# HKU-BAL/MegaPath-Nano

Hardware: AMD Instinct MI355X
Metric: Gbp/min ONT reads aligned+species-assigned vs RefSeq, 1/2/4/8 MI355X (higher is better)
Workload: dtype int32

## Files before the change

### megapath_nano_amd/csrc/map_kernels.h

```cpp
#pragma once
#include "mpn_common.h"
#include "map_types.h"

#include <type_traits>

namespace mpn {

__device__ __forceinline__ uint64_t hash64m(uint64_t key, uint64_t mask) {
    key = (~key + (key << 21)) & mask;
    key = key ^ key >> 24;
    key = ((key + (key << 3)) + (key << 8)) & mask;
    key = key ^ key >> 14;
    key = ((key + (key << 2)) + (key << 4)) & mask;
    key = key ^ key >> 28;
    key = (key + (key << 31)) & mask;
    return key;
}

constexpr int SKETCH_FAST_MAX_W = 32;

template <bool HASH64>
__device__ __forceinline__ uint64_t sketch_hash(uint64_t key, uint64_t mask) {
    if (HASH64) return hash64m(key, mask);
    uint32_t h = (uint32_t)key;
// ... 653 lines not shown
                int lo = 0, hi = 63;
#pragma unroll
                for (int step = 0; step < 6; ++step) {
                    const int mid = (lo + hi + 1) >> 1;
                    if (g[mid] <= p) lo = mid; else hi = mid - 1;
                }
                const uint64_t r = pos[ps[lo] + (p - g[lo])];
                const uint64_t y = yy[lo];
                const uint32_t q_pos = (uint32_t)y, q_span = (uint32_t)(y >> 32) & 0xff;
                const uint32_t rpos = (uint32_t)r >> 1;
                u128 a;
                if ((r & 1) == (q_pos & 1)) {
                    a.x = (r & 0xffffffff00000000ULL) | rpos;
                    a.y = (uint64_t)q_span << 32 | q_pos >> 1;
                } else {
                    a.x = 1ULL << 63 | (r & 0xffffffff00000000ULL) | rpos;
                    a.y = (uint64_t)q_span << 32 | (uint32_t)(qlen - ((int32_t)(q_pos >> 1) + 1 - (int32_t)q_span) - 1);
                }
                a.y |= y & (1ULL << 42);
                anchors[out + __popcll(km & ((1ULL << lane) - 1))] = a;
            }
            out += __popcll(km);
        }
        __builtin_amdgcn_wave_barrier();
    }
}

template <int NY>
__device__ __forceinline__ uint32_t sort_digit(const u128 &r, int pass) {
    return pass < NY ? (uint32_t)(r.y >> (8 * pass)) & 0xff : (uint32_t)(r.x >> (8 * (pass - NY))) & 0xff;
}

constexpr int WORK_SLOTS = 256;
__device__ __forceinline__ void add_work(unsigned long long *work, unsigned long long n) {
    if (work) atomicAdd(&work[blockIdx.x & (WORK_SLOTS - 1)], n);
}

struct SegSortLds {
    uint32_t hist[256], bins[256], wcnt[4][256];
    int skip;
};

template <int NY>
__device__ __forceinline__ void wg_radix_sort(SegSortLds &L, u128 *__restrict__ data, u128 *__restrict__ tmp, int64_t n,
                                              unsigned long long *__restrict__ work) {
    const int tid = threadIdx.x, lane = tid & 63, wv = tid >> 6;
    u128 *src = data, *dst = tmp;
    for (int pass = 0; pass < NY + 8; ++pass) {
        L.hist[tid] = 0;
        __syncthreads();
        for (int64_t i = tid; i < n; i += 256) atomicAdd(&L.hist[sort_digit<NY>(src[i], pass)], 1u);
        __syncthreads();
        if (tid == 0) L.skip = 0;
        __syncthreads();
        if (L.hist[tid] == (uint32_t)n) L.skip = 1;
        __syncthreads();
        if (L.skip) { __syncthreads(); continue; }
        if (tid == 0) add_work(work, (unsigned long long)n);
        {
            uint32_t v = L.hist[tid];
            L.bins[tid] = v;
            __syncthreads();
            for (int d = 1; d < 256; d <<= 1) {
                uint32_t a = tid >= d ? L.bins[tid - d] : 0;
                __syncthreads();
                L.bins[tid] += a;
// ... 559 lines not shown
                    max_f = best;
                    max_j = j0 - wl;
                }
                if (!tile_in_ring && elig && pj >= 0) {
                    if (pj >= win_lo) wt[pj & M] = i;
                    else { t[pj] = i; gmark = true; }
                }
                if (brk < 64) done = true;
                if (__ballot(gmark)) __builtin_amdgcn_fence(__ATOMIC_RELEASE, "workgroup");
                MPN_LDS_FENCE();
            }
            int32_t vprev = 0;
            if (max_j >= 0) vprev = max_j >= win_lo ? wv[max_j & M] : v[max_j];
            const int32_t vi = (max_j >= 0 && vprev > max_f) ? vprev : max_f;
            if (lane == li) { rf = max_f; rp = max_j >= 0 ? max_j + rel : -1; rv = vi; }
            if (lane == 0) {
                const int sl = i & M;
                *reinterpret_cast<uint4 *>(&ring[sl]) = make_uint4(ri, (uint32_t)qi, (uint32_t)max_f, (uint32_t)max_j);
                wv[sl] = vi; wt[sl] = 0;
            }
            MPN_LDS_FENCE();
            if (li == 63 || i == n - 1) {
                const int32_t k = (i & ~63) + lane;
                if (k <= i) { f[k] = rf; p[k] = rp; v[k] = rv; }
                const uint32_t carry = (uint32_t)__builtin_amdgcn_readlane((int)cx, 63);
                cx = (uint32_t)wave_scan_add((int)nstep) + carry; cx64 = nx64; cyl = nyl; cyh = nyh;
            }
        }
        __builtin_amdgcn_fence(__ATOMIC_RELEASE, "workgroup");
        __syncthreads();
    }
}

__global__ __launch_bounds__(64) void chain_ends_kernel(const int64_t *__restrict__ anchor_off, int n_reads, ChainParams cp,
                                                        const int32_t *__restrict__ F, const int32_t *__restrict__ P,
                                                        int32_t *__restrict__ T, const int32_t *__restrict__ V,
                                                        uint64_t *__restrict__ U, int32_t *__restrict__ n_ends) {
    const int lane = threadIdx.x;
    for (int read = blockIdx.x; read < n_reads; read += gridDim.x) {
        const int64_t base = anchor_off[read];
        const int64_t n = anchor_off[read + 1] - base;
        const int32_t *f = F + base, *p = P + base, *v = V + base;
        int32_t *t = T + base;
        uint64_t *u = U + base;
        for (int64_t i = lane; i < n; i += 64) t[i] = 0;
        __builtin_amdgcn_fence(__ATOMIC_RELEASE, "workgroup");
        __syncthreads();
        for (int64_t i = lane; i < n; i += 64) if (p[i] >= 0) t[p[i]] = 1;
        __builtin_amdgcn_fence(__ATOMIC_RELEASE, "workgroup");
        __syncthreads();
        int cnt = 0;
        for (int64_t i0 = 0; i0 < n; i0 += 64) {
            const int64_t i = i0 + lane;
            bool is_end = i < n && t[i] == 0 && v[i] >= cp.min_sc;
            uint64_t val = 0;
            if (is_end) {
                int64_t j = i;
                while (j >= 0 && f[j] < v[j]) j = p[j];
                if (j < 0) j = i;
                val = (uint64_t)(uint32_t)f[j] << 32 | (uint64_t)j;
            }
            const unsigned long long m = __ballot(is_end);
            if (is_end) u[cnt + __popcll(m & ((1ULL << lane) - 1))] = val;
            cnt += __popcll(m);
        }
        if (lane == 0) n_ends[read] = cnt;
        __syncthreads();
    }
}

__global__ __launch_bounds__(256) void chain_sort_ends_kernel(uint64_t *__restrict__ U, uint64_t *__restrict__ Utmp,
                                                              const int64_t *__restrict__ anchor_off,
                                                              const int32_t *__restrict__ n_ends, int n_reads) {
    __shared__ uint32_t hist[256];
    __shared__ uint32_t bins[256];
    __shared__ uint32_t wcnt[4][256];
    __shared__ int s_skip;
    const int tid = threadIdx.x, lane = tid & 63, wv = tid >> 6;
    for (int read = blockIdx.x; read < n_reads; read += gridDim.x) {
        const int64_t base = anchor_off[read];
        const int n = n_ends[read];
        if (n < 2) continue;
        uint64_t *src = U + base, *dst = Utmp + base;
        for (int pass = 0; pass < 8; ++pass) {
            hist[tid] = 0;
            __syncthreads();
            for (int i = tid; i < n; i += 256) atomicAdd(&hist[(uint32_t)(~src[i] >> (8 * pass)) & 0xff], 1u);
            __syncthreads();
            if (tid == 0) s_skip = 0;
            __syncthreads();
            if (hist[tid] == (uint32_t)n) s_skip = 1;
            __syncthreads();
            if (s_skip) { __syncthreads(); continue; }
            {
                uint32_t v = hist[tid];
                bins[tid] = v;
                __syncthreads();
                for (int d = 1; d < 256; d <<= 1) {
                    uint32_t a = tid >= d ? bins[tid - d] : 0;
                    __syncthreads();
                    bins[tid] += a;
                    __syncthreads();
                }
                uint32_t excl = bins[tid] - v;
                __syncthreads();
                bins[tid] = excl;
                __syncthreads();
            }
            for (int t0 = 0; t0 < n; t0 += 256) {
                const int i = t0 + tid;
                const bool act = i < n;
                uint64_t r = 0;
                uint32_t dg = 0;
                if (act) { r = src[i]; dg = (uint32_t)(~r >> (8 * pass)) & 0xff; }
                wcnt[0][tid] = 0; wcnt[1][tid] = 0; wcnt[2][tid] = 0; wcnt[3][tid] = 0;
                __syncthreads();
                unsigned long long same = __ballot(act);
#pragma unroll
                for (int b = 0; b < 8; ++b) {
                    unsigned long long m = __ballot((dg >> b) & 1);
                    same &= ((dg >> b) & 1) ? m : ~m;
                }
                const uint32_t rank = __popcll(same & ((1ULL << lane) - 1));
                if (act && rank == 0) wcnt[wv][dg] = __popcll(same);
                __syncthreads();
                if (act) {
                    uint32_t o = bins[dg] + rank;
                    for (int w2 = 0; w2 < wv; ++w2) o += wcnt[w2][dg];
                    dst[o] = r;
                }
                __syncthreads();
                bins[tid] += wcnt[0][tid] + wcnt[1][tid] + wcnt[2][tid] + wcnt[3][tid];
                __syncthreads();
            }
            uint64_t *sw = src; src = dst; dst = sw;
            __threadfence_block();
            __syncthreads();
        }
        if (src != U + base) for (int i = tid; i < n; i += 256) U[base + i] = src[i];
        __syncthreads();
    }
}

constexpr int BT_PAR_MIN = 16;

__global__ __launch_bounds__(64) void chain_backtrack_kernel(const u128 *__restrict__ anchors, const int64_t *__restrict__ anchor_off,
                                                             int n_reads, ChainParams cp, const int32_t *__restrict__ F,
                                                             const int32_t *__restrict__ P, int32_t *__restrict__ T,
                                                             int32_t *__restrict__ V, uint64_t *__restrict__ U,
                                                             const int32_t *__restrict__ n_ends, u128 *__restrict__ B,
                                                             uint64_t *__restrict__ Uc, unsigned long long *__restrict__ used,
                                                             int64_t *__restrict__ u_pos, int64_t *__restrict__ b_pos,
                                                             int32_t *__restrict__ n_chain, int64_t *__restrict__ n_chained,
                                                             ChainRec *__restrict__ Rc, int par_min) {
    __shared__ int s_k;
    __shared__ unsigned long long s_up, s_bp;
    const int lane = threadIdx.x;
    for (int read = blockIdx.x; read < n_reads; read += gridDim.x) {
        const int64_t base = anchor_off[read];
        const int64_t n = anchor_off[read + 1] - base;
        const u128 *a = anchors + base;
        const int32_t *f = F + base, *p = P + base;
        int32_t *t = T + base, *v = V + base;
        uint64_t *u = U + base;
        const int n_u = n_ends[read];
        if (n_u >= par_min) {
            for (int64_t i = lane; i < n; i += 64) t[i] = 0x7fffffff;
            __builtin_amdgcn_fence(__ATOMIC_RELEASE, "agent");
            __syncthreads();
            for (int e0 = 0; e0 < n_u; e0 += 64) {
                const int e = e0 + lane;
                if (e < n_u) {
                    int32_t j = (int32_t)u[e];
                    while (j >= 0) { const int32_t nj = p[j]; if (atomicMin(&t[j], e) < e) break; j = nj; }
                }
            }
            __builtin_amdgcn_fence(__ATOMIC_ACQ_REL, "agent");
            __syncthreads();
            int k_run = 0, nv_run = 0;
            for (int e0 = 0; e0 < n_u; e0 += 64) {
                const int e = e0 + lane;
                int cnt = 0;
                if (e < n_u) {
                    const uint64_t ui = u[e];
                    int32_t j = p[(int32_t)ui];
                    cnt = 1;
                    while (j >= 0) { const int32_t tj = t[j], nj = p[j]; if (tj != e) break; ++cnt; j = nj; }
                    const bool keep = cnt >= cp.min_cnt && (j < 0 || (int32_t)(ui >> 32) - f[j] >= cp.min_sc);
                    if (!keep) cnt = 0;
                    v[e] = cnt;
                }
                k_run += __builtin_amdgcn_readlane(wave_scan_add(cnt > 0 ? 1 : 0), 63);
                nv_run += __builtin_amdgcn_readlane(wave_scan_add(cnt), 63);
// ... 78 lines not shown
        const int k = s_k;
        u128 *b = B + s_bp;
        uint64_t *uc = Uc + s_up;
        ChainRec *rc = Rc + s_up;
        int off = 0;
        for (int c = 0; c < k; ++c) {
            const int ni = (int32_t)u[c];
            int ml = 0, bl = 0;
            for (int j = lane; j < ni; j += 64) {
                const u128 cur = a[v[off + (ni - j - 1)]];
                b[off + j] = cur;
                const int span = (int)(cur.y >> 32 & 0xff);
                if (j == 0) { ml += span; bl += span; }
                else {
                    const u128 prev = a[v[off + (ni - j)]];
                    const int tl = (int32_t)cur.x - (int32_t)prev.x, ql = (int32_t)cur.y - (int32_t)prev.y;
                    bl += tl > ql ? tl : ql;
                    ml += tl > span && ql > span ? span : tl < ql ? tl : ql;
                }
            }
            ml = __builtin_amdgcn_readlane(wave_scan_add(ml), 63);
            bl = __builtin_amdgcn_readlane(wave_scan_add(bl), 63);
            if (lane == 0) {
                const u128 first = a[v[off + ni - 1]], last = a[v[off]];
                rc[c] = ChainRec{first.x, first.y, last.x, last.y, ml, bl};
            }
            off += ni;
        }
        for (int c = lane; c < k; c += 64) uc[c] = u[c];
        __syncthreads();
    }
}

__global__ __launch_bounds__(256) void idx_bucket_hist_kernel(const u128 *__restrict__ mz, int64_t n, int shift, unsigned long long *__restrict__ hist) {
    for (int64_t i = (int64_t)blockIdx.x * blockDim.x + threadIdx.x; i < n; i += (int64_t)gridDim.x * blockDim.x)
        atomicAdd(&hist[(mz[i].x >> 8) >> shift], 1ULL);
}

__global__ __launch_bounds__(256) void idx_bucket_scatter_kernel(const u128 *__restrict__ mz, int64_t n, int shift,
                                                                 unsigned long long *__restrict__ cursor, u128 *__restrict__ out) {
    for (int64_t i = (int64_t)blockIdx.x * blockDim.x + threadIdx.x; i < n; i += (int64_t)gridDim.x * blockDim.x) {
        u128 r = mz[i];
        r.x >>= 8;
        const unsigned long long p = atomicAdd(&cursor[r.x >> shift], 1ULL);
        out[p] = r;
    }
}

__global__ __launch_bounds__(256) void idx_flag_count_kernel(const u128 *__restrict__ rec, int64_t n, int64_t *__restrict__ block_cnt) {
    __shared__ int s[256];
    const int64_t base = (int64_t)blockIdx.x * 2048;
    int c = 0;
    for (int k = 0; k < 8; ++k) {
        const int64_t i = base + k * 256 + threadIdx.x;
        if (i < n && (i == 0 || rec[i].x != rec[i - 1].x)) ++c;
    }
    s[threadIdx.x] = c;
    __syncthreads();
    for (int d = 128; d; d >>= 1) { if (threadIdx.x < d) s[threadIdx.x] += s[threadIdx.x + d]; __syncthreads(); }
    if (threadIdx.x == 0) block_cnt[blockIdx.x] = s[0];
}

__global__ __launch_bounds__(256) void idx_emit_kernel(const u128 *__restrict__ rec, int64_t n, const int64_t *__restrict__ block_off,
                                                       uint64_t *__restrict__ keys, int64_t *__restrict__ key_off,
                                                       uint64_t *__restrict__ pos) {
    __shared__ int s[256];
// ... 77 lines not shown
```

### megapath_nano_amd/csrc/mapper.hip

```cpp
#include "map_kernels.h"
#include "mapper_internal.h"
#include "../../include/mpn_map.h"

#include <algorithm>
#include <mutex>
#include <string.h>
#include <time.h>
#include <sys/stat.h>
#include <string>
#include <vector>

namespace mpn {

hipError_t stream_sync(hipStream_t st) {
    struct Ev {
        hipEvent_t e = nullptr;
        ~Ev() { if (e) (void)hipEventDestroy(e); }
    };
    static thread_local Ev ev;
    hipError_t rc;
    if (!ev.e && (rc = hipEventCreateWithFlags(&ev.e, hipEventDisableTiming)) != hipSuccess) return rc;
    if ((rc = hipEventRecord(ev.e, st)) != hipSuccess) return rc;
    unsigned int us = 20;
    for (;;) {
// ... 189 lines not shown
int sketch_reads(int k, int w, int n, const uint8_t *d_seqs, const int64_t *d_off, const int32_t *d_len, const int32_t *h_len, ReadSketch &sk,
                 StreamLease &st) {
    EvTimer ev(st);
    sk.valid = false;
    if (sketch_device(d_seqs, d_off, d_len, h_len, n, k, w, 0, sk.mz_off, sk.mz, &sk.n_mz, st, &ev)) return -1;
    MPN_HIP_CHECK(stream_sync(st));
    ev.resolve();
    sk.k = k; sk.w = w; sk.valid = true;
    return 0;
}

int seed_chain_device(const mpn_index *idx, const mpn_map_opt *opt, int n, const uint8_t *d_seqs, const int64_t *d_off,
                      const int32_t *d_len, const int32_t *h_len, SeedChainOut &o, StreamLease &st, const ReadSketch *pre) {
    int64_t n_mz = 0;
    DevBuf<int64_t> mz_off;
    DevBuf<u128> mz;
    EvTimer ev(st);
    if (pre && pre->valid && pre->k == idx->k && pre->w == idx->w) {
        mz_off.p = pre->mz_off.p; mz_off.n = pre->mz_off.n; mz_off.owned = false;
        mz.p = pre->mz.p; mz.n = pre->mz.n; mz.owned = false;
        n_mz = pre->n_mz;
    } else if (sketch_device(d_seqs, d_off, d_len, h_len, n, idx->k, idx->w, 0, mz_off, mz, &n_mz, st, &ev)) return -1;
    g_stats[1] += n_mz;
    int32_t mid_occ = opt->mid_occ > 0 ? opt->mid_occ : mpn_index_mid_occ(idx, opt->mid_occ_frac);
    if (mid_occ > (1 << 25)) {
        const int32_t top = mpn_index_mid_occ(idx, 1e-30f);
        if (top > 0) mid_occ = std::min(mid_occ, top);
    }
    DevBuf<int32_t> occ;
    DevBuf<int64_t> pos_start, rel_off, full_off, n_blk, blk_base;
    DevBuf<unsigned long long> span_sum;
    {
        const size_t N = (size_t)n, o1 = (N + 1) * 8, o2 = o1 + N * 8, o3 = o2 + N * 8, o4 = o3 + N * 8, o5 = o4 + N * 4, o6 = (o5 + N * 4 + 7) & ~(size_t)7;
        o.tables_bytes = o6 + (size_t)(2 + WORK_SLOTS) * 8;
        if (o.tables.alloc(o.tables_bytes)) return -1;
        auto view = [&](auto &buf, size_t off, size_t count) { buf.release(); buf.p = reinterpret_cast<decltype(buf.p)>(o.tables.p + off); buf.n = count; buf.owned = false; };
        view(o.n_anchor, 0, N + 1); view(o.n_chained, o1, N); view(o.u_pos, o2, N); view(o.b_pos, o3, N);
        view(o.n_chain, o4, N); view(o.rep_len, o5, N); view(o.used, o6, 2 + WORK_SLOTS);
    }
    if (occ.alloc(n_mz) || pos_start.alloc(n_mz) || rel_off.alloc(n_mz) || full_off.alloc((size_t)n + 1) ||
        n_blk.alloc((size_t)n + 1) || blk_base.alloc((size_t)n + 1) || span_sum.alloc(n) || o.anchor_off.alloc((size_t)n + 1))
        return -1;
    if (n_mz > 0) {
        hipLaunchKernelGGL(seed_lookup_kernel, dim3(grid_1d(n_mz, 256)), dim3(256), 0, st, (const u128 *)idx->kv.p,
                           idx->n_keys, (const int64_t *)idx->bucket_start.p, idx->bucket_shift, mz.p, n_mz, mid_occ, occ.p, pos_start.p);
        MPN_HIP_CHECK(hipGetLastError());
        ev.mark(11, 35);
    }
    hipLaunchKernelGGL(seed_prefix_kernel, dim3(std::max(1, std::min(n, 256 * 32))), dim3(64), 0, st, mz.p, mz_off.p, n, occ.p, rel_off.p,
                       o.n_anchor.p, o.rep_len.p, span_sum.p, n_blk.p);
    MPN_HIP_CHECK(hipGetLastError());
    hipLaunchKernelGGL(scan_i64x2_kernel, dim3(2), dim3(1024), 0, st, (const int64_t *)o.n_anchor.p, full_off.p, n, (const int64_t *)n_blk.p, blk_base.p, n);
    MPN_HIP_CHECK(hipGetLastError());
    int64_t n_full = 0;
    if (read_i64(full_off.p + n, &n_full, st)) return -1;
    g_stats[2] += n_full;
    const int64_t nb_cap = n_mz / 64 + n + 1;
    DevBuf<unsigned long long> keep;
    DevBuf<int64_t> blk_kept, blk_off;
    DevBuf<int32_t> blk_read, order;
    DevBuf<unsigned int> next_read;
    DevBuf<unsigned int> n_list, seg_counters;
    DevBuf<unsigned long long> read_kept;
    if (next_read.alloc(4) || order.alloc(n) || keep.alloc((size_t)(n_full / 64 + nb_cap + 8)) || blk_kept.alloc((size_t)nb_cap + 1) || blk_off.alloc((size_t)nb_cap + 2) ||
        blk_read.alloc((size_t)nb_cap + 1) || n_list.alloc(4) || seg_counters.alloc(4) || read_kept.alloc(n))
        return -1;
    {
        ZeroList z{};
        zero_list_push(z, next_read.p, 4 * sizeof(unsigned int));
        zero_list_push(z, blk_kept.p, ((size_t)nb_cap + 1) * 8);
        zero_list_push(z, o.used.p, o.used.n * sizeof(unsigned long long));
// ... 77 lines not shown
                           (const unsigned int *)n_list.p, lists.cap[0], o.used.p + 2);
        hipLaunchKernelGGL(anchor_bitonic_list_kernel<BITONIC_MID>, dim3(256 * 4), dim3(256), 0, st, o.anchors.p, (const SortSeg *)lists.seg[1],
                           (const unsigned int *)n_list.p + 1, lists.cap[1], o.used.p + 2);
        hipLaunchKernelGGL(seg_sort_list_kernel<4>, dim3(256 * 4), dim3(256), 0, st, o.anchors.p, tmp.p, (const SortSeg *)lists.seg[2],
                           (const unsigned int *)n_list.p + 2, lists.cap[2], o.used.p + 2);
        MPN_HIP_CHECK(hipGetLastError());
        ev.mark(12, 49);
    }
    ChainParams cp;
    cp.max_dist_x = opt->max_gap; cp.max_dist_y = opt->max_gap; cp.bw = opt->bw; cp.max_skip = opt->max_chain_skip;
    cp.max_iter = opt->max_chain_iter; cp.min_cnt = opt->min_cnt; cp.min_sc = opt->min_chain_score;
    const int g = std::max(1, std::min(n, 256 * 32));
    const int64_t n_pieces = (n_a + COMPACT_PIECE - 1) / COMPACT_PIECE;
    DevBuf<int64_t> kept, piece_kept, piece_off;
    DevBuf<float> avg_qspan;
    if (kept.alloc((size_t)n + 1) || o.c_off.alloc((size_t)n + 1) || avg_qspan.alloc(n) || piece_kept.alloc((size_t)n_pieces + 1) ||
        piece_off.alloc((size_t)n_pieces + 1))
        return -1;
    const int gp = (int)std::max<int64_t>(1, std::min<int64_t>(n_pieces, 256 * 64));
    if (n_a > 0) {
        hipLaunchKernelGGL(anchor_compact_kernel<false>, dim3(gp), dim3(64), 0, st, (const u128 *)o.anchors.p, (const int64_t *)o.anchor_off.p, n, n_a,
                           cp.max_dist_x, cp.min_cnt, piece_kept.p, read_kept.p, (const int64_t *)nullptr, (u128 *)nullptr);
        MPN_HIP_CHECK(hipGetLastError());
    }
    hipLaunchKernelGGL(anchor_compact_finish_kernel, dim3((n + 255) / 256), dim3(256), 0, st, (const int64_t *)o.n_anchor.p, n,
                       (const unsigned long long *)read_kept.p, (const unsigned long long *)span_sum.p, kept.p, avg_qspan.p);
    hipLaunchKernelGGL(scan_i64x2_kernel, dim3(2), dim3(1024), 0, st, (const int64_t *)kept.p, o.c_off.p, n, (const int64_t *)piece_kept.p, piece_off.p, (int)n_pieces);
    MPN_HIP_CHECK(hipGetLastError());
    int64_t n_c = 0;
    if (read_i64(o.c_off.p + n, &n_c, st)) return -1;
    g_stats[45] += n_c;
    DevBuf<int32_t> F, P, T, V;
    DevBuf<uint64_t> Utmp;
    if (F.alloc(n_c) || P.alloc(n_c) || T.alloc(n_c) || V.alloc(n_c) || o.u.alloc(n_c) || Utmp.alloc(n_c) || o.chained.alloc(n_c) ||
        o.recs.alloc((size_t)(n_c / std::max(1, opt->min_cnt)) + 1))
        return -1;
    u128 *ca = tmp.p;
    if (n_a > 0) {
        hipLaunchKernelGGL(anchor_compact_kernel<true>, dim3(gp), dim3(64), 0, st, (const u128 *)o.anchors.p, (const int64_t *)o.anchor_off.p, n, n_a,
                           cp.max_dist_x, cp.min_cnt, (int64_t *)nullptr, (unsigned long long *)nullptr, (const int64_t *)piece_off.p, ca);
        MPN_HIP_CHECK(hipGetLastError());
    }
    ev.mark(46);
    DevBuf<ChainSeg> seg_big, seg_small;
    static const int chain_item = []() { const char *e = getenv("MPN_CHAIN_ITEM"); return e ? std::min(CHAIN_BIG, std::max(16, atoi(e))) : CHAIN_ITEM; }();
    if (seg_big.alloc((size_t)n_c / CHAIN_BIG + (size_t)n + 1) || seg_small.alloc((size_t)n_c / chain_item + (size_t)n + 1)) return -1;
    hipLaunchKernelGGL(chain_segments_kernel, dim3(g), dim3(64), 0, st, (const u128 *)ca, (const int64_t *)o.c_off.p, n, cp, avg_qspan.p, 1, seg_big.p,
                       seg_small.p, seg_counters.p, chain_item);
    MPN_HIP_CHECK(hipGetLastError());
    ev.mark(13);
    hipLaunchKernelGGL(chain_dp_kernel, dim3(256 * 32), dim3(64), 0, st, (const u128 *)ca, (const int64_t *)o.c_off.p, (const float *)avg_qspan.p,
                       (const ChainSeg *)seg_big.p, (const ChainSeg *)seg_small.p, seg_counters.p, cp, F.p, P.p, T.p, V.p);
    MPN_HIP_CHECK(hipGetLastError());
    ev.mark(13, 37);
    hipLaunchKernelGGL(chain_ends_kernel, dim3(g), dim3(64), 0, st, (const int64_t *)o.c_off.p, n, cp, F.p, P.p, T.p, V.p, o.u.p, o.n_ends.p);
    MPN_HIP_CHECK(hipGetLastError());
    hipLaunchKernelGGL(chain_sort_ends_kernel, dim3(std::max(1, std::min(n, 256 * 8))), dim3(256), 0, st, o.u.p, Utmp.p,
                       (const int64_t *)o.c_off.p, o.n_ends.p, n);
    MPN_HIP_CHECK(hipGetLastError());
    o.u_compact.p = Utmp.p; o.u_compact.n = Utmp.n; o.u_compact.owned = Utmp.owned; Utmp.p = nullptr; Utmp.n = 0;
    static const int bt_par_min = []() { const char *e = getenv("MPN_BT_PAR_MIN"); return e ? std::max(1, atoi(e)) : BT_PAR_MIN; }();
    hipLaunchKernelGGL(chain_backtrack_kernel, dim3(g), dim3(64), 0, st, (const u128 *)ca, (const int64_t *)o.c_off.p, n, cp, F.p, P.p, T.p, V.p,
                       o.u.p, o.n_ends.p, o.chained.p, o.u_compact.p, o.used.p, o.u_pos.p, o.b_pos.p, o.n_chain.p, o.n_chained.p, o.recs.p, bt_par_min);
    MPN_HIP_CHECK(hipGetLastError());
    ev.mark(14);
    MPN_HIP_CHECK(stream_sync(st));
    ev.resolve();
    return 0;
}

int download_chains(int n, SeedChainOut &o, HostChains &h, PoolBuf &pin_u, PoolBuf &pin_b, StreamLease &st, int mode) {
    const bool with_anchors = mode == 2;
    h.n_anchor.resize((size_t)n);
    h.n_chain.resize(n); h.n_chained.resize(n); h.rep_len.resize(n); h.u_pos.resize(n); h.b_pos.resize(n);
    unsigned long long used[2 + WORK_SLOTS] = {0};
    {
        const size_t N = (size_t)n;
        const size_t o1 = (N + 1) * 8, o2 = o1 + N * 8, o3 = o2 + N * 8, o4 = o3 + N * 8, o5 = o4 + N * 4, o6 = (o5 + N * 4 + 7) & ~(size_t)7;
        char *pn = (char *)tl_pin.get(o.tables_bytes + 64);
        if (!pn) { set_error("pinned scratch allocation failed"); return -1; }
        MPN_HIP_CHECK(hipMemcpyAsync(pn, o.tables.p, o.tables_bytes, hipMemcpyDeviceToHost, st));
        MPN_HIP_CHECK(stream_sync(st));
        memcpy(h.n_anchor.data(), pn, N * 8); memcpy(h.n_chained.data(), pn + o1, N * 8);
        memcpy(h.u_pos.data(), pn + o2, N * 8); memcpy(h.b_pos.data(), pn + o3, N * 8);
        memcpy(h.n_chain.data(), pn + o4, N * 4); memcpy(h.rep_len.data(), pn + o5, N * 4);
        memcpy(used, pn + o6, sizeof(used));
    }
    for (int k = 0; k < WORK_SLOTS; ++k) g_stats[44] += (int64_t)used[2 + k];
    ++g_stats[32];
    h.n_pool_chains = (int64_t)used[0];
    if (mode == 0) { h.u_all = nullptr; h.rec_all = nullptr; h.b_all = nullptr; }
    else if (with_anchors) {
        if (pin_u.ensure((size_t)used[0] * 8 + 16) || pin_b.ensure((size_t)used[1] * 16 + 16)) return -1;
        if (o.u_compact.download(pin_u.as<uint64_t>(), (size_t)used[0], st) || o.chained.download(pin_b.as<u128>(), (size_t)used[1], st)) return -1;
        h.u_all = pin_u.as<uint64_t>(); h.b_all = pin_b.as<u128>();
    } else {
        const size_t rec_bytes = ((size_t)used[0] * sizeof(ChainRec) + 15) & ~(size_t)15;
        if (pin_u.ensure(rec_bytes + (size_t)used[0] * 8 + 16)) return -1;
        h.rec_all = pin_u.as<ChainRec>();
        h.u_all = reinterpret_cast<const uint64_t *>(reinterpret_cast<const char *>(pin_u.p) + rec_bytes);
        h.b_all = nullptr;
        if (o.recs.download(const_cast<ChainRec *>(h.rec_all), (size_t)used[0], st) || o.u_compact.download(const_cast<uint64_t *>(h.u_all), (size_t)used[0], st)) return -1;
    }
    h.chain_off.assign((size_t)n + 1, 0);
    h.b_off.assign((size_t)n + 1, 0);
    for (int i = 0; i < n; ++i) { h.chain_off[i + 1] = h.chain_off[i] + h.n_chain[i]; h.b_off[i + 1] = h.b_off[i] + h.n_chained[i]; }
    MPN_HIP_CHECK(stream_sync(st));
    return 0;
}

void HostChains::read_chains(int i, uint64_t *uo, u128 *bo) const {
    const int nc = n_chain[i];
    if (nc == 0) return;
    const uint64_t *u = u_all + u_pos[i];
    const u128 *b = b_all + b_pos[i];
    std::vector<std::pair<std::pair<uint64_t, uint64_t>, int>> w(nc);
    int64_t k = 0;
    for (int c = 0; c < nc; ++c) { w[c] = {{b[k].x, (uint64_t)k << 32 | (uint32_t)c}, c}; k += (int32_t)u[c]; }
    std::sort(w.begin(), w.end());
    int64_t kk = 0;
    for (int c = 0; c < nc; ++c) {
// ... 526 lines not shown
```

### megapath_nano_amd/csrc/mapper_internal.h

```cpp
#pragma once
#include "mpn_common.h"
#include "map_types.h"
#include "queue_lease.h"

#include <atomic>
#include <chrono>
#include <time.h>
#include <mutex>
#include <stdint.h>
#include <stdlib.h>
#include <string.h>
#include <string>
#include <vector>

struct mpn_map_opt_s;


struct mpn_index {
    int k = 15, w = 10;
    int32_t n_seq = 0;
    std::vector<std::string> names;
    std::vector<int32_t> lens;
    std::vector<int64_t> seq_off;
    std::vector<uint32_t> h_seq2;
// ... 18 lines not shown
struct SeedChainOut {
    int64_t n_anchors = 0;
    DevBuf<unsigned char> tables;
    size_t tables_bytes = 0;
    DevBuf<int64_t> n_anchor;
    DevBuf<int64_t> anchor_off, c_off, n_chained, u_pos, b_pos;
    DevBuf<int32_t> rep_len, n_ends, n_chain;
    DevBuf<u128> anchors, chained;
    DevBuf<uint64_t> u, u_compact;
    DevBuf<ChainRec> recs;
    DevBuf<unsigned long long> used;
};

struct ReadSketch {
    DevBuf<int64_t> mz_off;
    DevBuf<u128> mz;
    int64_t n_mz = 0;
    int k = 0, w = 0;
    bool valid = false;
};

struct HostChains {
    std::vector<int64_t> n_anchor, chain_off, b_off;
    std::vector<int64_t> n_chained, u_pos, b_pos;
    std::vector<int32_t> n_chain, rep_len;
    const uint64_t *u_all = nullptr;
    const u128 *b_all = nullptr;
    const ChainRec *rec_all = nullptr;
    int64_t n_pool_chains = 0;
    void read_chains(int i, uint64_t *u_out, u128 *b_out) const;
    void chain_order(int i, int32_t *order, int64_t *src) const;
};

constexpr int MPN_NSTATS = 77;
constexpr int STAT_LEASE_WAIT = 65;
constexpr int STAT_SIDE_LEASED = 66, STAT_SIDE_OWN = 67;
constexpr int STAT_TILE_CLASS = 68, STAT_TILE_GIVEUPS = 72;
constexpr int STAT_WALK_WAVE = 73, STAT_EV_WALK_LONG = 74, STAT_WALK_WAVE_FAILED = 75;
constexpr int STAT_K_TAGS = 76;
extern thread_local int64_t g_stats[MPN_NSTATS];

void pack_2bit(const uint8_t *codes, int64_t n, std::vector<uint32_t> &words, std::vector<int64_t> &ns, std::vector<int64_t> &ne);

hipError_t stream_sync(hipStream_t st);

struct QueueStreams {
    LeasePool pool;
    std::vector<hipStream_t> st;
    explicit QueueStreams(int q) : pool(q), st((size_t)q, nullptr) {}
};
QueueStreams *queue_streams(int dev);

class StreamLease {
  public:
    explicit StreamLease(QueueStreams *qs) : qs_(qs) {}
    explicit StreamLease(hipStream_t fixed) : fixed_(fixed) {}
    StreamLease(const StreamLease &) = delete;
    StreamLease &operator=(const StreamLease &) = delete;
    ~StreamLease() { release(); }
    hipStream_t get() {
        if (!qs_) return fixed_;
        if (n_ == 0) n_ = qs_->pool.acquire(1, id_, &g_stats[STAT_LEASE_WAIT]);
        return qs_->st[(size_t)id_[0]];
    }
    operator hipStream_t() { return get(); }
    int try_extra(int k, hipStream_t *out) {
        if (!qs_ || n_ == 0) return 0;
        const int got = qs_->pool.try_acquire(std::min(k, 3 - n_), id_ + n_);
        for (int i = 0; i < got; ++i) out[i] = qs_->st[(size_t)id_[n_ + i]];
        n_ += got;
        return got;
    }
// ... 111 lines not shown
```

### megapath_nano_amd/mapper.py

```python
import ctypes as ct
import os

import numpy as np

from . import _ffi


class MapOpt(ct.Structure):
    _fields_ = [('k', ct.c_int32), ('w', ct.c_int32), ('mid_occ_frac', ct.c_float), ('mid_occ', ct.c_int32),
                ('max_gap', ct.c_int32), ('bw', ct.c_int32), ('max_chain_skip', ct.c_int32), ('max_chain_iter', ct.c_int32),
                ('min_cnt', ct.c_int32), ('min_chain_score', ct.c_int32), ('mask_level', ct.c_float),
                ('pri_ratio', ct.c_float), ('best_n', ct.c_int32), ('max_join_long', ct.c_int32),
                ('max_join_short', ct.c_int32), ('min_join_flank_sc', ct.c_int32), ('min_join_flank_ratio', ct.c_float),
                ('a', ct.c_int32), ('b', ct.c_int32), ('q', ct.c_int32), ('e', ct.c_int32), ('q2', ct.c_int32),
                ('e2', ct.c_int32), ('sc_ambi', ct.c_int32), ('zdrop', ct.c_int32), ('zdrop_inv', ct.c_int32),
                ('end_bonus', ct.c_int32), ('min_dp_max', ct.c_int32), ('min_ksw_len', ct.c_int32),
                ('max_clip_ratio', ct.c_float), ('max_sw_mat', ct.c_int64), ('with_cigar', ct.c_int32),
                ('seed', ct.c_uint32), ('host_threads', ct.c_int32), ('out_sam', ct.c_int32), ('out_tags', ct.c_int32)]


TAG_CS, TAG_CS_LONG, TAG_MD, TAG_EQX = 1, 2, 4, 8


COL_NAMES = ('read_idx', 'qs', 'qe', 'rev', 'rid', 'rs', 're', 'mlen', 'blen', 'mapq', 'nm', 'as_', 'primary')
# ... 850 lines not shown
    anchor_off, cig_pos, compact = c(anchor_off, np.int64), c(cig_pos, np.int64), c(compact, np.uint32)
    anchors, hits, wins = c(anchors, np.uint64).reshape(-1, 2), c(hits, np.int32).reshape(-1, 15), c(wins, np.int32).reshape(-1, 13)
    n = len(anchor_off) - 1
    assert n >= 0 and len(anchors) == (int(anchor_off[-1]) if n else 0) and len(cig_pos) == len(wins)
    n_hits = len(hits)
    pool_cap = int(np.maximum(wins[:, 12].astype(np.int64), 0).sum())
    out = np.zeros((n_hits + 1, 25), dtype=np.int64)
    pool = np.zeros(pool_cap + 1, dtype=np.uint32)
    splits = np.zeros((n_hits + 1, 8), dtype=np.int64)
    used, n_splits = ct.c_int64(0), ct.c_int64(0)
    rc = lib.mpn_stitch_batch(n, anchor_off.ctypes.data, anchors.ctypes.data, n_hits, hits.ctypes.data, len(wins), wins.ctypes.data,
                              cig_pos.ctypes.data, len(compact), compact.ctypes.data, int(min_cnt), int(grid_cap), out.ctypes.data, pool_cap,
                              pool.ctypes.data, ct.addressof(used), splits.ctypes.data, ct.addressof(n_splits))
    _ffi.check(rc, 'mpn_stitch_batch')
    return out[:n_hits], pool[:used.value], splits[:n_splits.value]


STAT_NAMES = {0: 'bases', 1: 'minimizers', 2: 'anchors', 3: 'chains', 4: 'dp_jobs', 5: 'dp_cells', 6: 'alignments',
              7: 'dp_rounds', 8: 'second_pass_jobs', 10: 'ev_sketch_ns', 11: 'ev_seed_ns', 12: 'ev_sort_ns',
              13: 'ev_chain_dp_ns', 14: 'ev_chain_bt_ns', 15: 'ev_ext_dp_ns', 25: 'ev_ext_bt_ns', 26: 'ev_ext_ztest_ns',
              16: 'wall_h2d_ns', 17: 'wall_seed_chain_ns', 18: 'wall_d2h_chains_ns', 19: 'wall_host_hits_ns',
              20: 'wall_host_plan_ns', 21: 'wall_ext_stage_ns', 22: 'wall_host_stitch_ns', 23: 'wall_host_final_ns',
              24: 'wall_total_ns', 27: 'wall_ext_host_prep_ns', 28: 'wall_ext_enqueue_ns', 29: 'wall_ext_gpu_wait_ns',
              30: 'wall_ext_finish_ns', 9: 'ev_ext_strip_ns', 31: 'strip_cells', 32: 'sub_batches',
              33: 'k_sketch_count_ns', 34: 'k_sketch_fill_ns', 35: 'k_seed_lookup_ns', 36: 'k_seed_fill_ns',
              37: 'k_chain_dp_ns', 38: 'k_strip16_ns', 39: 'k_strip32_ns', 40: 'k_strip64_ns', 41: 'strip16_cells',
              42: 'strip32_cells', 43: 'strip64_cells', 44: 'sort_records_moved', 45: 'anchors_kept', 46: 'k_compact_ns', 47: 'k_sort_msd_ns', 48: 'k_sort_chunk_ns', 49: 'k_sort_radix_ns',
              50: 'k_seed_filter_ns', 51: 'anchors_emitted', 52: 'k_finish_ns', 53: 'cigar_ops', 54: 'k_stitch_ns', 55: 'k_plan_ns', 56: 'k_layout_ns', 57: 'k_xstrip_ns', 58: 'xstrip_cells', 59: 'anchors_squeezed', 60: 'workers_shed', 61: 'workers', 62: 'k_hit_select_ns', 63: 'reads_hits_on_host',
              64: 'tile_windows', 65: 'wall_lease_wait_ns', 66: 'ext_groups_side_leased', 67: 'ext_groups_side_own',
              68: 'tile_windows_1w_s16', 69: 'tile_windows_s4_nw8', 70: 'tile_windows_s8_nw4', 71: 'tile_windows_s4_nw16',
              72: 'tile_wait_giveups',
              73: 'walk_wave_windows', 74: 'ev_ext_walk_long_ns',
              75: 'walk_wave_failed',
              76: 'k_tags_ns'}


def last_stats():
    n = max(STAT_NAMES) + 1
    s = np.zeros(n, dtype=np.int64)
    _bind().mpn_map_last_stats_ex(s.ctypes.data, n)
    return {name: int(s[i]) for i, name in STAT_NAMES.items()}
```

Before: 14.67.

## Fuse chain end-finding, sorting and backtrack into one LDS-resident kernel for small reads

Adds a 256-thread kernel that, for each read whose anchor count fits a shared-memory cap, finds chain ends, sorts their keys (bitonic sort in LDS, or radix sort when there are many), assigns anchor ownership and emits the chains, all in one pass. Predecessor links are stored as 16-bit distances in LDS. The kernel runs in two size classes with different dynamic LDS sizes, so small reads can keep more blocks resident per CU. The existing three-kernel global path skips reads handled this way and returns early when no read is left for it. The cost is extra LDS pressure, more code paths, and reads whose link distance exceeds the 16-bit range must still take the global path.

Result: no change. 14.65 (-0.2%).

```diff
diff --git a/megapath_nano_amd/csrc/map_kernels.h b/megapath_nano_amd/csrc/map_kernels.h
--- a/megapath_nano_amd/csrc/map_kernels.h
+++ b/megapath_nano_amd/csrc/map_kernels.h
@@ -709,6 +709,7 @@
 }
 
 constexpr int WORK_SLOTS = 256;
+constexpr int USED_BT_COUNT = 2 + WORK_SLOTS, USED_WORDS = USED_BT_COUNT + 2;
 __device__ __forceinline__ void add_work(unsigned long long *work, unsigned long long n) {
     if (work) atomicAdd(&work[blockIdx.x & (WORK_SLOTS - 1)], n);
 }
@@ -1334,14 +1335,19 @@
     }
 }
 
+__device__ __forceinline__ bool bt_lds_takes(int64_t n, int lds_cap) { return lds_cap > 0 && n <= (int64_t)lds_cap; }
+
 __global__ __launch_bounds__(64) void chain_ends_kernel(const int64_t *__restrict__ anchor_off, int n_reads, ChainParams cp,
                                                         const int32_t *__restrict__ F, const int32_t *__restrict__ P,
                                                         int32_t *__restrict__ T, const int32_t *__restrict__ V,
-                                                        uint64_t *__restrict__ U, int32_t *__restrict__ n_ends) {
+                                                        uint64_t *__restrict__ U, int32_t *__restrict__ n_ends, int lds_cap,
+                                                        const unsigned long long *__restrict__ bt_global) {
     const int lane = threadIdx.x;
+    if (lds_cap > 0 && *bt_global == 0) return;
     for (int read = blockIdx.x; read < n_reads; read += gridDim.x) {
         const int64_t base = anchor_off[read];
         const int64_t n = anchor_off[read + 1] - base;
+        if (bt_lds_takes(n, lds_cap)) continue;
         const int32_t *f = F + base, *p = P + base, *v = V + base;
         int32_t *t = T + base;
         uint64_t *u = U + base;
@@ -1371,76 +1377,85 @@
     }
 }
 
+constexpr int CHAIN_SORT_LDS_WORDS = 256 + 256 + 4 * 256 + 1;
+
+__device__ __forceinline__ void chain_sort_ends_read(uint64_t *__restrict__ u_read, uint64_t *__restrict__ tmp_read, int n,
+                                                     uint32_t *__restrict__ lds) {
+    uint32_t *hist = lds, *bins = lds + 256, *wcnt = lds + 512;
+    int *s_skip = reinterpret_cast<int *>(lds + 1536);
+    const int tid = threadIdx.x, lane = tid & 63, wv = tid >> 6;
+    uint64_t *src = u_read, *dst = tmp_read;
+    for (int pass = 0; pass < 8; ++pass) {
+        hist[tid] = 0;
+        __syncthreads();
+        for (int i = tid; i < n; i += 256) atomicAdd(&hist[(uint32_t)(~src[i] >> (8 * pass)) & 0xff], 1u);
+        __syncthreads();
+        if (tid == 0) *s_skip = 0;
+        __syncthreads();
+        if (hist[tid] == (uint32_t)n) *s_skip = 1;
+        __syncthreads();
+        if (*s_skip) { __syncthreads(); continue; }
+        {
+            uint32_t v = hist[tid];
+            bins[tid] = v;
+            __syncthreads();
+            for (int d = 1; d < 256; d <<= 1) {
+                uint32_t a = tid >= d ? bins[tid - d] : 0;
+                __syncthreads();
+                bins[tid] += a;
+                __syncthreads();
+            }
+            uint32_t excl = bins[tid] - v;
+            __syncthreads();
+            bins[tid] = excl;
+            __syncthreads();
+        }
+        for (int t0 = 0; t0 < n; t0 += 256) {
+            const int i = t0 + tid;
+            const bool act = i < n;
+            uint64_t r = 0;
+            uint32_t dg = 0;
+            if (act) { r = src[i]; dg = (uint32_t)(~r >> (8 * pass)) & 0xff; }
+            wcnt[tid] = 0; wcnt[256 + tid] = 0; wcnt[512 + tid] = 0; wcnt[768 + tid] = 0;
+            __syncthreads();
+            unsigned long long same = __ballot(act);
+#pragma unroll
+            for (int b = 0; b < 8; ++b) {
+                unsigned long long m = __ballot((dg >> b) & 1);
+                same &= ((dg >> b) & 1) ? m : ~m;
+            }
+            const uint32_t rank = __popcll(same & ((1ULL << lane) - 1));
+            if (act && rank == 0) wcnt[wv * 256 + dg] = __popcll(same);
+            __syncthreads();
+            if (act) {
+                uint32_t o = bins[dg] + rank;
+                for (int w2 = 0; w2 < wv; ++w2) o += wcnt[w2 * 256 + dg];
+                dst[o] = r;
+            }
+            __syncthreads();
+            bins[tid] += wcnt[tid] + wcnt[256 + tid] + wcnt[512 + tid] + wcnt[768 + tid];
+            __syncthreads();
+        }
+        uint64_t *sw = src; src = dst; dst = sw;
+        __threadfence_block();
+        __syncthreads();
+    }
+    if (src != u_read) for (int i = tid; i < n; i += 256) u_read[i] = src[i];
+    __syncthreads();
+}
+
 __global__ __launch_bounds__(256) void chain_sort_ends_kernel(uint64_t *__restrict__ U, uint64_t *__restrict__ Utmp,
                                                               const int64_t *__restrict__ anchor_off,
-                                                              const int32_t *__restrict__ n_ends, int n_reads) {
-    __shared__ uint32_t hist[256];
-    __shared__ uint32_t bins[256];
-    __shared__ uint32_t wcnt[4][256];
-    __shared__ int s_skip;
-    const int tid = threadIdx.x, lane = tid & 63, wv = tid >> 6;
+                                                              const int32_t *__restrict__ n_ends, int n_reads, int lds_cap,
+                                                              const unsigned long long *__restrict__ bt_global) {
+    __shared__ uint32_t lds[CHAIN_SORT_LDS_WORDS];
+    if (lds_cap > 0 && *bt_global == 0) return;
     for (int read = blockIdx.x; read < n_reads; read += gridDim.x) {
         const int64_t base = anchor_off[read];
+        if (bt_lds_takes(anchor_off[read + 1] - base, lds_cap)) continue;
         const int n = n_ends[read];
         if (n < 2) continue;
-        uint64_t *src = U + base, *dst = Utmp + base;
-        for (int pass = 0; pass < 8; ++pass) {
-            hist[tid] = 0;
-            __syncthreads();
-            for (int i = tid; i < n; i += 256) atomicAdd(&hist[(uint32_t)(~src[i] >> (8 * pass)) & 0xff], 1u);
-            __syncthreads();
-            if (tid == 0) s_skip = 0;
-            __syncthreads();
-            if (hist[tid] == (uint32_t)n) s_skip = 1;
-            __syncthreads();
-            if (s_skip) { __syncthreads(); continue; }
-            {
-                uint32_t v = hist[tid];
-                bins[tid] = v;
-                __syncthreads();
-                for (int d = 1; d < 256; d <<= 1) {
-                    uint32_t a = tid >= d ? bins[tid - d] : 0;
-                    __syncthreads();
-                    bins[tid] += a;
-                    __syncthreads();
-                }
-                uint32_t excl = bins[tid] - v;
-                __syncthreads();
-                bins[tid] = excl;
-                __syncthreads();
-            }
-            for (int t0 = 0; t0 < n; t0 += 256) {
-                const int i = t0 + tid;
-                const bool act = i < n;
-                uint64_t r = 0;
-                uint32_t dg = 0;
-                if (act) { r = src[i]; dg = (uint32_t)(~r >> (8 * pass)) & 0xff; }
-                wcnt[0][tid] = 0; wcnt[1][tid] = 0; wcnt[2][tid] = 0; wcnt[3][tid] = 0;
-                __syncthreads();
-                unsigned long long same = __ballot(act);
-#pragma unroll
-                for (int b = 0; b < 8; ++b) {
-                    unsigned long long m = __ballot((dg >> b) & 1);
-                    same &= ((dg >> b) & 1) ? m : ~m;
-                }
-                const uint32_t rank = __popcll(same & ((1ULL << lane) - 1));
-                if (act && rank == 0) wcnt[wv][dg] = __popcll(same);
-                __syncthreads();
-                if (act) {
-                    uint32_t o = bins[dg] + rank;
-                    for (int w2 = 0; w2 < wv; ++w2) o += wcnt[w2][dg];
-                    dst[o] = r;
-                }
-                __syncthreads();
-                bins[tid] += wcnt[0][tid] + wcnt[1][tid] + wcnt[2][tid] + wcnt[3][tid];
-                __syncthreads();
-            }
-            uint64_t *sw = src; src = dst; dst = sw;
-            __threadfence_block();
-            __syncthreads();
-        }
-        if (src != U + base) for (int i = tid; i < n; i += 256) U[base + i] = src[i];
-        __syncthreads();
+        chain_sort_ends_read(U + base, Utmp + base, n, lds);
     }
 }
 
@@ -1454,13 +1469,17 @@
                                                              uint64_t *__restrict__ Uc, unsigned long long *__restrict__ used,
                                                              int64_t *__restrict__ u_pos, int64_t *__restrict__ b_pos,
                                                              int32_t *__restrict__ n_chain, int64_t *__restrict__ n_chained,
-                                                             ChainRec *__restrict__ Rc, int par_min) {
+                                                             ChainRec *__restrict__ Rc, int par_min, int lds_cap,
+                                                             unsigned long long *__restrict__ bt_global) {
     __shared__ int s_k;
     __shared__ unsigned long long s_up, s_bp;
     const int lane = threadIdx.x;
+    if (lds_cap > 0 && *bt_global == 0) return;
     for (int read = blockIdx.x; read < n_reads; read += gridDim.x) {
         const int64_t base = anchor_off[read];
         const int64_t n = anchor_off[read + 1] - base;
+        if (bt_lds_takes(n, lds_cap)) continue;
+        if (lds_cap == 0 && n > 0 && lane == 0) atomicAdd(bt_global, 1ULL);
         const u128 *a = anchors + base;
         const int32_t *f = F + base, *p = P + base;
         int32_t *t = T + base, *v = V + base;
@@ -1605,6 +1624,169 @@
     }
 }
 
+constexpr int BT_LDS_KEYS = 1024;
+constexpr int BT_LDS_CAP_SMALL = 7168, BT_LDS_CAP_LARGE = 24576;
+constexpr int BT_LDS_MAX_LINK = 65534;
+constexpr uint16_t BT_NO_LINK = 0xffff;
+constexpr size_t bt_lds_bytes(int cap) { return (size_t)BT_LDS_KEYS * 8 + (size_t)cap * 6; }
+static_assert((size_t)BT_LDS_KEYS * 8 >= (size_t)CHAIN_SORT_LDS_WORDS * 4, "the radix passes borrow the key area");
+static_assert(3 * (bt_lds_bytes(BT_LDS_CAP_SMALL) + 1280) <= 160 * 1024 && bt_lds_bytes(BT_LDS_CAP_LARGE) + 1280 <= 160 * 1024, "LDS of a CU");
+
+__global__ __launch_bounds__(256) void chain_bt_lds_kernel(const u128 *__restrict__ anchors, const int64_t *__restrict__ anchor_off, int n_reads,
+                                                           ChainParams cp, const int32_t *__restrict__ F, const int32_t *__restrict__ P,
+                                                           int32_t *__restrict__ V, uint64_t *__restrict__ U, uint64_t *__restrict__ Utmp,
+                                                           int32_t *__restrict__ n_ends, u128 *__restrict__ B, uint64_t *__restrict__ Uc,
+                                                           unsigned long long *__restrict__ used, int64_t *__restrict__ u_pos,
+                                                           int64_t *__restrict__ b_pos, int32_t *__restrict__ n_chain,
+                                                           int64_t *__restrict__ n_chained, ChainRec *__restrict__ Rc, int cap_lo, int cap_hi,
+                                                           int lds_cap, unsigned long long *__restrict__ bt_count) {
+    extern __shared__ __attribute__((aligned(16))) uint8_t bt_lds[];
+    __shared__ int s_cnt, s_k, s_nv, s_w[8];
+    __shared__ unsigned long long s_up, s_bp;
+    uint64_t *keys = reinterpret_cast<uint64_t *>(bt_lds);
+    uint32_t *own = reinterpret_cast<uint32_t *>(bt_lds + (size_t)BT_LDS_KEYS * 8);
+    uint16_t *dist = reinterpret_cast<uint16_t *>(own + cap_hi);
+    const int tid = threadIdx.x, lane = tid & 63, wv = tid >> 6;
+    auto prev = [&](int32_t j) -> int32_t { const uint16_t d = dist[j]; return d == BT_NO_LINK ? -1 : j - (int32_t)d; };
+    for (int read = blockIdx.x; read < n_reads; read += gridDim.x) {
+        const int64_t base = anchor_off[read];
+        const int64_t n64 = anchor_off[read + 1] - base;
+        if (n64 > (int64_t)lds_cap) {
+            if (cap_lo < 0 && tid == 0) atomicAdd(&bt_count[1], 1ULL);
+            continue;
+        }
+        if (n64 <= (int64_t)cap_lo || n64 > (int64_t)cap_hi) continue;
+        const int32_t n = (int32_t)n64;
+        if (n == 0) {
+            if (tid == 0) { n_ends[read] = 0; n_chain[read] = 0; n_chained[read] = 0; u_pos[read] = 0; b_pos[read] = 0; }
+            continue;
+        }
+        const u128 *a = anchors + base;
+        const int32_t *f = F + base, *p = P + base;
+        int32_t *v = V + base;
+        uint64_t *u = U + base;
+        if (tid == 0) { s_cnt = 0; s_k = 0; s_nv = 0; atomicAdd(&bt_count[0], 1ULL); }
+        for (int32_t i = tid; i < n; i += 256) {
+            const int32_t pi = p[i];
+            dist[i] = pi >= 0 && pi < i ? (uint16_t)(i - pi) : BT_NO_LINK;
+            own[i] = 0;
+        }
+        __syncthreads();
+        for (int32_t i = tid; i < n; i += 256) { const uint16_t d = dist[i]; if (d != BT_NO_LINK) own[i - (int32_t)d] = 1; }
+        __syncthreads();
+        for (int32_t i = tid; i < n; i += 256) {
+            if (own[i] != 0 || v[i] < cp.min_sc) continue;
+            int32_t j = i;
+            while (j >= 0 && f[j] < v[j]) j = prev(j);
+            if (j < 0) j = i;
+            const uint64_t key = (uint64_t)(uint32_t)f[j] << 32 | (uint64_t)(uint32_t)j;
+            const int pos = atomicAdd(&s_cnt, 1);
+            if (pos < BT_LDS_KEYS) keys[pos] = key; else u[pos] = key;
+        }
+        __syncthreads();
+        const int n_u = s_cnt;
+        const bool keys_in_lds = n_u <= BT_LDS_KEYS;
+        if (!keys_in_lds) {
+            for (int i = tid; i < BT_LDS_KEYS; i += 256) u[i] = keys[i];
+            __threadfence_block();
+            __syncthreads();
+            chain_sort_ends_read(u, Utmp + base, n_u, reinterpret_cast<uint32_t *>(keys));
+        } else if (n_u > 1) {
+            int m = 2;
+            while (m < n_u) m <<= 1;
+            for (int i = n_u + tid; i < m; i += 256) keys[i] = 0;
+            __syncthreads();
+            for (int k = 2; k <= m; k <<= 1)
+                for (int jj = k >> 1; jj > 0; jj >>= 1) {
+                    for (int i = tid; i < m; i += 256) {
+                        const int x = i ^ jj;
+                        if (x > i) {
+                            const uint64_t ka = keys[i], kb = keys[x];
+                            if ((i & k) == 0 ? ka < kb : ka > kb) { keys[i] = kb; keys[x] = ka; }
+                        }
+                    }
+                    __syncthreads();
+                }
+        }
+        auto key_of = [&](int e) -> uint64_t { return keys_in_lds ? keys[e] : u[e]; };
+        for (int32_t i = tid; i < n; i += 256) own[i] = 0x7fffffffu;
+        __syncthreads();
+        for (int e = tid; e < n_u; e += 256) {
+            int32_t j = (int32_t)(uint32_t)key_of(e);
+            while (j >= 0) { const int32_t nj = prev(j); if (atomicMin(&own[j], (uint32_t)e) < (uint32_t)e) break; j = nj; }
+        }
+        __syncthreads();
+        for (int e = tid; e < n_u; e += 256) {
+            const uint64_t ui = key_of(e);
+            int32_t j = prev((int32_t)(uint32_t)ui);
+            int cnt = 1;
+            while (j >= 0 && own[j] == (uint32_t)e) { ++cnt; j = prev(j); }
+            const bool keep = cnt >= cp.min_cnt && (j < 0 || (int32_t)(ui >> 32) - f[j] >= cp.min_sc);
+            if (!keep) cnt = 0;
+            v[e] = cnt;
+            if (cnt > 0) { atomicAdd(&s_k, 1); atomicAdd(&s_nv, cnt); }
+        }
+        __syncthreads();
+        if (tid == 0) {
+            const int k = s_k, nv = s_nv;
+            n_ends[read] = n_u;
+            n_chain[read] = k;
+            n_chained[read] = nv;
+            s_up = k ? atomicAdd(&used[0], (unsigned long long)k) : 0ULL;
+            s_bp = nv ? atomicAdd(&used[1], (unsigned long long)nv) : 0ULL;
+            u_pos[read] = (int64_t)s_up;
+            b_pos[read] = (int64_t)s_bp;
+        }
+        __syncthreads();
+        u128 *b = B + s_bp;
+        uint64_t *uc = Uc + s_up;
+        ChainRec *rc = Rc + s_up;
+        int k_run = 0, nv_run = 0;
+        for (int e0 = 0; e0 < n_u; e0 += 256) {
+            const int e = e0 + tid;
+            const int cnt = e < n_u ? v[e] : 0;
+            const int incl = wave_scan_add(cnt), kin = wave_scan_add(cnt > 0 ? 1 : 0);
+            if (lane == 63) { s_w[wv] = incl; s_w[4 + wv] = kin; }
+            __syncthreads();
+            int pre_c = 0, pre_k = 0, tot_c = 0, tot_k = 0;
+#pragma unroll
+            for (int w = 0; w < 4; ++w) {
+                const int c = s_w[w], k = s_w[4 + w];
+                if (w < wv) { pre_c += c; pre_k += k; }
+                tot_c += c; tot_k += k;
+            }
+            if (cnt > 0) {
+                const int kidx = k_run + pre_k + kin - 1, off = nv_run + pre_c + incl - cnt;
+                const uint64_t ui = key_of(e);
+                int32_t j = (int32_t)(uint32_t)ui;
+                u128 nxt = a[j];
+                const u128 last = nxt;
+                int ml = 0, bl = 0;
+                b[off + cnt - 1] = nxt;
+                for (int q = cnt - 2; q >= 0; --q) {
+                    j = prev(j);
+                    const u128 cur = a[j];
+                    b[off + q] = cur;
+                    const int span = (int)(nxt.y >> 32 & 0xff);
+                    const int tl = (int32_t)nxt.x - (int32_t)cur.x, ql = (int32_t)nxt.y - (int32_t)cur.y;
+                    bl += tl > ql ? tl : ql;
+                    ml += tl > span && ql > span ? span : tl < ql ? tl : ql;
+                    nxt = cur;
+                }
+                const int span0 = (int)(nxt.y >> 32 & 0xff);
+                ml += span0; bl += span0;
+                j = prev(j);
+                const uint64_t sc = j < 0 ? ui >> 32 : (ui >> 32) - (uint64_t)f[j];
+                uc[kidx] = sc << 32 | (uint32_t)cnt;
+                rc[kidx] = ChainRec{nxt.x, nxt.y, last.x, last.y, ml, bl};
+            }
+            k_run += tot_k; nv_run += tot_c;
+            __syncthreads();
+        }
+        __syncthreads();
+    }
+}
+
 __global__ __launch_bounds__(256) void idx_bucket_hist_kernel(const u128 *__restrict__ mz, int64_t n, int shift, unsigned long long *__restrict__ hist) {
     for (int64_t i = (int64_t)blockIdx.x * blockDim.x + threadIdx.x; i < n; i += (int64_t)gridDim.x * blockDim.x)
         atomicAdd(&hist[(mz[i].x >> 8) >> shift], 1ULL);
diff --git a/megapath_nano_amd/csrc/mapper.hip b/megapath_nano_amd/csrc/mapper.hip
--- a/megapath_nano_amd/csrc/mapper.hip
+++ b/megapath_nano_amd/csrc/mapper.hip
@@ -245,11 +245,11 @@
     DevBuf<unsigned long long> span_sum;
     {
         const size_t N = (size_t)n, o1 = (N + 1) * 8, o2 = o1 + N * 8, o3 = o2 + N * 8, o4 = o3 + N * 8, o5 = o4 + N * 4, o6 = (o5 + N * 4 + 7) & ~(size_t)7;
-        o.tables_bytes = o6 + (size_t)(2 + WORK_SLOTS) * 8;
+        o.tables_bytes = o6 + (size_t)USED_WORDS * 8;
         if (o.tables.alloc(o.tables_bytes)) return -1;
         auto view = [&](auto &buf, size_t off, size_t count) { buf.release(); buf.p = reinterpret_cast<decltype(buf.p)>(o.tables.p + off); buf.n = count; buf.owned = false; };
         view(o.n_anchor, 0, N + 1); view(o.n_chained, o1, N); view(o.u_pos, o2, N); view(o.b_pos, o3, N);
-        view(o.n_chain, o4, N); view(o.rep_len, o5, N); view(o.used, o6, 2 + WORK_SLOTS);
+        view(o.n_chain, o4, N); view(o.rep_len, o5, N); view(o.used, o6, USED_WORDS);
     }
     if (occ.alloc(n_mz) || pos_start.alloc(n_mz) || rel_off.alloc(n_mz) || full_off.alloc((size_t)n + 1) ||
         n_blk.alloc((size_t)n + 1) || blk_base.alloc((size_t)n + 1) || span_sum.alloc(n) || o.anchor_off.alloc((size_t)n + 1))
@@ -393,8 +393,9 @@
     g_stats[45] += n_c;
     DevBuf<int32_t> F, P, T, V;
     DevBuf<uint64_t> Utmp;
+    const size_t chain_cap = (size_t)(n_c / std::max(1, opt->min_cnt)) + 1;
     if (F.alloc(n_c) || P.alloc(n_c) || T.alloc(n_c) || V.alloc(n_c) || o.u.alloc(n_c) || Utmp.alloc(n_c) || o.chained.alloc(n_c) ||
-        o.recs.alloc((size_t)(n_c / std::max(1, opt->min_cnt)) + 1))
+        o.u_compact.alloc(chain_cap) || o.recs.alloc(chain_cap))
         return -1;
     u128 *ca = tmp.p;
     if (n_a > 0) {
@@ -414,15 +415,31 @@
                        (const ChainSeg *)seg_big.p, (const ChainSeg *)seg_small.p, seg_counters.p, cp, F.p, P.p, T.p, V.p);
     MPN_HIP_CHECK(hipGetLastError());
     ev.mark(13, 37);
-    hipLaunchKernelGGL(chain_ends_kernel, dim3(g), dim3(64), 0, st, (const int64_t *)o.c_off.p, n, cp, F.p, P.p, T.p, V.p, o.u.p, o.n_ends.p);
+    static const bool bt_lds_on = []() { const char *e = getenv("MPN_BT_LDS"); return !(e && !strcmp(e, "off")); }();
+    static const int bt_lds_cap = []() { const char *e = getenv("MPN_BT_LDS_CAP"); return e ? std::min(BT_LDS_CAP_LARGE, std::max(1, atoi(e))) : BT_LDS_CAP_LARGE; }();
+    const int lds_cap = bt_lds_on && cp.max_iter <= BT_LDS_MAX_LINK ? bt_lds_cap : 0;
+    unsigned long long *bt_count = o.used.p + USED_BT_COUNT;
+    if (lds_cap > 0) {
+        MPN_HIP_CHECK(hipFuncSetAttribute((const void *)chain_bt_lds_kernel, hipFuncAttributeMaxDynamicSharedMemorySize, (int)bt_lds_bytes(BT_LDS_CAP_LARGE)));
+        const int cap_small = std::min(lds_cap, BT_LDS_CAP_SMALL);
+        for (int cls = 0; cls < (lds_cap > cap_small ? 2 : 1); ++cls) {
+            const int lo = cls ? cap_small : -1, hi = cls ? lds_cap : cap_small;
+            hipLaunchKernelGGL(chain_bt_lds_kernel, dim3(g), dim3(256), bt_lds_bytes(hi), st, (const u128 *)ca, (const int64_t *)o.c_off.p, n, cp,
+                               (const int32_t *)F.p, (const int32_t *)P.p, V.p, o.u.p, Utmp.p, o.n_ends.p, o.chained.p, o.u_compact.p, o.used.p,
+                               o.u_pos.p, o.b_pos.p, o.n_chain.p, o.n_chained.p, o.recs.p, lo, hi, lds_cap, bt_count);
+            MPN_HIP_CHECK(hipGetLastError());
+        }
+    }
+    hipLaunchKernelGGL(chain_ends_kernel, dim3(g), dim3(64), 0, st, (const int64_t *)o.c_off.p, n, cp, F.p, P.p, T.p, V.p, o.u.p, o.n_ends.p, lds_cap,
+                       (const unsigned long long *)bt_count + 1);
     MPN_HIP_CHECK(hipGetLastError());
     hipLaunchKernelGGL(chain_sort_ends_kernel, dim3(std::max(1, std::min(n, 256 * 8))), dim3(256), 0, st, o.u.p, Utmp.p,
-                       (const int64_t *)o.c_off.p, o.n_ends.p, n);
-    MPN_HIP_CHECK(hipGetLastError());
-    o.u_compact.p = Utmp.p; o.u_compact.n = Utmp.n; o.u_compact.owned = Utmp.owned; Utmp.p = nullptr; Utmp.n = 0;
+                       (const int64_t *)o.c_off.p, o.n_ends.p, n, lds_cap, (const unsigned long long *)bt_count + 1);
+    MPN_HIP_CHECK(hipGetLastError());
     static const int bt_par_min = []() { const char *e = getenv("MPN_BT_PAR_MIN"); return e ? std::max(1, atoi(e)) : BT_PAR_MIN; }();
     hipLaunchKernelGGL(chain_backtrack_kernel, dim3(g), dim3(64), 0, st, (const u128 *)ca, (const int64_t *)o.c_off.p, n, cp, F.p, P.p, T.p, V.p,
-                       o.u.p, o.n_ends.p, o.chained.p, o.u_compact.p, o.used.p, o.u_pos.p, o.b_pos.p, o.n_chain.p, o.n_chained.p, o.recs.p, bt_par_min);
+                       o.u.p, o.n_ends.p, o.chained.p, o.u_compact.p, o.used.p, o.u_pos.p, o.b_pos.p, o.n_chain.p, o.n_chained.p, o.recs.p, bt_par_min,
+                       lds_cap, bt_count + 1);
     MPN_HIP_CHECK(hipGetLastError());
     ev.mark(14);
     MPN_HIP_CHECK(stream_sync(st));
@@ -434,7 +451,7 @@
     const bool with_anchors = mode == 2;
     h.n_anchor.resize((size_t)n);
     h.n_chain.resize(n); h.n_chained.resize(n); h.rep_len.resize(n); h.u_pos.resize(n); h.b_pos.resize(n);
-    unsigned long long used[2 + WORK_SLOTS] = {0};
+    unsigned long long used[USED_WORDS] = {0};
     {
         const size_t N = (size_t)n;
         const size_t o1 = (N + 1) * 8, o2 = o1 + N * 8, o3 = o2 + N * 8, o4 = o3 + N * 8, o5 = o4 + N * 4, o6 = (o5 + N * 4 + 7) & ~(size_t)7;
@@ -448,6 +465,7 @@
         memcpy(used, pn + o6, sizeof(used));
     }
     for (int k = 0; k < WORK_SLOTS; ++k) g_stats[44] += (int64_t)used[2 + k];
+    g_stats[STAT_BT_READS_LDS] += (int64_t)used[USED_BT_COUNT]; g_stats[STAT_BT_READS_GLOBAL] += (int64_t)used[USED_BT_COUNT + 1];
     ++g_stats[32];
     h.n_pool_chains = (int64_t)used[0];
     if (mode == 0) { h.u_all = nullptr; h.rec_all = nullptr; h.b_all = nullptr; }
diff --git a/megapath_nano_amd/csrc/mapper_internal.h b/megapath_nano_amd/csrc/mapper_internal.h
--- a/megapath_nano_amd/csrc/mapper_internal.h
+++ b/megapath_nano_amd/csrc/mapper_internal.h
@@ -74,12 +74,13 @@
     void chain_order(int i, int32_t *order, int64_t *src) const;
 };
 
-constexpr int MPN_NSTATS = 77;
+constexpr int MPN_NSTATS = 79;
 constexpr int STAT_LEASE_WAIT = 65;
 constexpr int STAT_SIDE_LEASED = 66, STAT_SIDE_OWN = 67;
 constexpr int STAT_TILE_CLASS = 68, STAT_TILE_GIVEUPS = 72;
 constexpr int STAT_WALK_WAVE = 73, STAT_EV_WALK_LONG = 74, STAT_WALK_WAVE_FAILED = 75;
 constexpr int STAT_K_TAGS = 76;
+constexpr int STAT_BT_READS_LDS = 77, STAT_BT_READS_GLOBAL = 78;
 extern thread_local int64_t g_stats[MPN_NSTATS];
 
 void pack_2bit(const uint8_t *codes, int64_t n, std::vector<uint32_t> &words, std::vector<int64_t> &ns, std::vector<int64_t> &ne);
diff --git a/megapath_nano_amd/mapper.py b/megapath_nano_amd/mapper.py
--- a/megapath_nano_amd/mapper.py
+++ b/megapath_nano_amd/mapper.py
@@ -906,7 +906,8 @@
               72: 'tile_wait_giveups',
               73: 'walk_wave_windows', 74: 'ev_ext_walk_long_ns',
               75: 'walk_wave_failed',
-              76: 'k_tags_ns'}
+              76: 'k_tags_ns',
+              77: 'bt_reads_lds', 78: 'bt_reads_global'}
 
 
 def last_stats():
```
